# zhb94430/RayTracer-Utah

Hardware: AMD Instinct MI355X
Metric: Mrays/sec at 1920x1080 (the reference's primary + secondary + shadow rays of the frames rendered / wall time; batched throughput: config.frames_in_flight frames with their own cameras per launch sequence — one frame alone: config.single_frame) (higher is better)
Workload: dtype f32

## Files before the change

### raytracer-utah_amd/csrc/render_impl.h

```cpp
#ifndef RTU_RENDER_IMPL_H_INCLUDED
#define RTU_RENDER_IMPL_H_INCLUDED
#include "rtu_intersect.h"

namespace {

#define TEXD ((TEX & 1) != 0)
#define SMPD ((TEX & 2) != 0)
#define BATD ((TEX & 4) != 0)
#define GID ((TEX & 8) != 0)
#define CNTD ((TEX & 16) != 0)
#ifndef RTU_OCC_PRIMARY
#define RTU_OCC_PRIMARY __attribute__((amdgpu_waves_per_eu(4, 4)))
#endif
#ifndef RTU_OCC_PRIMARY_S
#define RTU_OCC_PRIMARY_S __attribute__((amdgpu_waves_per_eu(5, 5)))
#endif
#ifndef RTU_OCC_TRACE
#define RTU_OCC_TRACE __attribute__((amdgpu_waves_per_eu(5, 5)))
#endif
#ifndef RTU_OCC_WALK
#define RTU_OCC_WALK __attribute__((amdgpu_waves_per_eu(3, 3)))
#endif
#ifndef RTU_OCC_CONSUME
#define RTU_OCC_CONSUME
// ... 336 lines not shown
                const int hmid = hit ? as_const(s.nodes)[h.node].material_id : -1;
                a.gi_h[ho] = make_float4(h.p.x, h.p.y, h.p.z, h.z);
                a.gi_h[ho + a.gi_total] = make_float4(h.N.x, h.N.y, h.N.z, __uint_as_float((hit ? 1u : 0u) | (h.front ? 2u : 0u) | ((uint32_t)(hmid + 1) << 2)));
                a.gi_h[ho + 2u * (size_t)a.gi_total] = make_float4(ray.dir.x, ray.dir.y, ray.dir.z, __uint_as_float(smp.key));
                if (TEXD) a.gi_h[ho + 3u * (size_t)a.gi_total] = make_float4(h.uvw.x, h.uvw.y, h.uvw.z, 0.0f);
                RTU_BYTES(TEXD ? 64u : 48u);
            }
        }
        return;
    }
    if (valid) {
        float ox = 0.5f, oy = 0.5f;
        if (smp.on) {
            smp.key = sample_key((uint32_t)x + (uint32_t)a.frame.width * (uint32_t)y, a.sample_index + sidx);
            ox = a.pix_off_x[sidx];
            oy = a.pix_off_y[sidx];
            const float sampleX = (float)rand31(smp.key, RTU_DRAW_LENS) / RTU_RAND_MAX_F;
            const float sampleTheta = (float)rand31(smp.key, RTU_DRAW_LENS + 1u) / RTU_THETA_DIV;
            float sn, cs;
            portable_sincos(sampleTheta, sn, cs);
            const float rad = sqrtf((sampleX * a.frame.dof) * a.frame.dof);
            const float camOffsetX = rad * cs, camOffsetY = rad * sn;
            ray.p = (ray.p + ld3(a.frame.lens_up) * camOffsetY) + ld3(a.frame.lens_right) * camOffsetX;
        }
        f3 cp = (cam_origin + cam_u * ((float)x + ox)) + cam_v * ((float)y + oy);
        ray.dir = norm3(cp - ray.p);
        RTU_CNT(prim);
        bool hit = false;
        const unsigned units0 = CNTD ? cnt.t_inner4 * 2u + cnt.t_tri : 0u;
        if (!(a.dbg & 4u)) hit = trace<STACK, STATS, !STATS, DEFER, COOP, TEXD, CNTD>(s, ray, false, h, stk, cnt, deferred, stride, lds_nodes, skip, rects);
        if (CNTD) walk_units = cnt.t_inner4 * 2u + cnt.t_tri - units0;
        if (!deferred && leader) {
            if (!hit) {
                f3 bg = background_sample<TEXD>(s, x, y);
                if (!(a.dbg & 16u)) a.out[pix] = make_float4(bg.x, bg.y, bg.z, h.z);
                RTU_BYTES(16u);
            } else {
                RTU_CNT(prim_hit);
                mid = as_const(s.nodes)[h.node].material_id;
                if (mid < 0) { a.out[pix] = make_float4(1.0f, 1.0f, 1.0f, h.z); RTU_BYTES(16u); }
                else want = true;
            }
            if (GID) {
                a.gi_h[pix] = make_float4(h.p.x, h.p.y, h.p.z, h.z);
                a.gi_h[pix + a.gi_total] = make_float4(h.N.x, h.N.y, h.N.z, __uint_as_float((want ? 1u : 0u) | (h.front ? 2u : 0u) | ((uint32_t)(mid + 1) << 2)));
                a.gi_h[pix + 2u * (size_t)a.gi_total] = make_float4(ray.dir.x, ray.dir.y, ray.dir.z, __uint_as_float(smp.key));
                if (TEXD) a.gi_h[pix + 3u * (size_t)a.gi_total] = make_float4(h.uvw.x, h.uvw.y, h.uvw.z, 0.0f);
                RTU_BYTES(TEXD ? 64u : 48u);
                want = false;
            }
        }
    }
    if (GID) return;
    uint32_t info = 0;
    if (want) info = make_info<TEX>(a, mid, a.frame.max_bounce, h.front, ray.dir, h.p, h.N, h.uvw, smp);
    if (!STATS && INLINE_SHADE && !(a.dbg & 2048u) && __any(want && !(info & (RTU_FI_MAIN | RTU_FI_C)))) {
        const bool tryI = want && !(info & (RTU_FI_MAIN | RTU_FI_C));
        uint32_t lit = ~0u;
        bool ok = false;
        if (tryI) ok = shadows_inline<TEX>(a, info, h.p, lit, cnt);
        if (tryI && ok) {
            f3 direct = mk3(0, 0, 0);
            if (info & RTU_FI_SH) {
                const f3 cam_pos = BATD ? ld3(a.cam[sidx].pos) : ld3(a.frame.cam_pos);
                direct = direct_light<false, TEX>(a, info, h.p, h.N, h.uvw, cam_pos, direct, [&](uint32_t j) { return ((lit >> j) & 1u) ? 1.0f : 0.0f; });
            }
            a.out[pix] = make_float4(direct.x, direct.y, direct.z, h.z);
            RTU_BYTES(16u);
            want = false;
        }
    }
    if (!(a.dbg & 8u)) append_root<TEX>(a, want, shard, info, h.p, h.N, pix, ray.dir, h.z, h.uvw, cnt, !DEFER && !STATS);
    if (CNTD && !DEFER && !COOP && (a.dbg & 131072u) && valid) a.out[pix].x = (float)walk_units;
}

template <int STACK, bool STATS, int TEX>
__device__ __forceinline__ void primary_stage1(const KernelArgs& a, uint32_t n_tiles) {
    const Stamp stamp(a, RTU_TL_PRIMARY);
    __shared__ uint32_t s_stack_all[STATS ? 4 * STACK * 64 : 4];
    uint32_t* stk = s_stack_all + (STATS ? (threadIdx.x >> 6) * (STACK * 64) + (threadIdx.x & 63u) : 0);
    const uint32_t lane = threadIdx.x & 63u;
    Counters cnt = {};
    const uint32_t wave = (uint32_t)__builtin_amdgcn_readfirstlane((int)(threadIdx.x >> 6));
    for (uint32_t btile = blockIdx.x * 4u + wave; btile < n_tiles; btile += gridDim.x * 4u) {
        uint32_t sidx = (SMPD || BATD) ? btile / a.tiles_per_image : 0u;
        uint32_t tile = btile - sidx * a.tiles_per_image;
        bool lane_on = true;
        if constexpr (SMPD) {
            if (a.act_list != nullptr) {
                sidx = btile / a.act_n;
                const RTU_CONST uint32_t* ent = as_const(reinterpret_cast<const uint32_t*>(a.act_list)) + 4u * (size_t)(btile - sidx * a.act_n);
                tile = ent[0];
                lane_on = (((unsigned long long)ent[3] << 32 | ent[2]) >> lane) & 1ull;
            }
        }
        const uint32_t band_local = tile / a.tiles_x;
        const uint32_t tx = tile - band_local * a.tiles_x;
        const int x = (int)(tx * 8 + (lane & 7));
        const int ly = (int)(band_local * RTU_BAND_ROWS + (lane >> 3));
        const int y = (int)((band_local * a.frame.shard_count + a.frame.shard_rank) * RTU_BAND_ROWS + (lane >> 3));
        const bool valid = x < a.frame.width && y < a.frame.height && lane_on;
        const uint32_t pix = ((SMPD || BATD) ? sidx * a.batch_pixels : 0u) + (uint32_t)ly * (uint32_t)a.frame.width + (uint32_t)x;
        if (!STATS && !SMPD && !GID && a.occ != nullptr) {
            const uint32_t w = as_const(a.occ)[(size_t)sidx * a.occ_words + (tile >> 5)];
            if (!((w >> (tile & 31u)) & 1u)) {
                if (valid) {
                    const f3 bg = background_sample<TEXD>(a.scene, x, y);
                    a.out[pix] = make_float4(bg.x, bg.y, bg.z, RTU_BIGFLOAT);
                    RTU_BYTES(16u);
                    if (CNTD) cnt.t_rays++;
                }
                if (CNTD && lane == 0) cnt.t_bytes += 4u;
                continue;
            }
        }
        const uint32_t shard = btile % RTU_SHARDS;
        bool deferred;
        primary_pixel<STACK, STATS, !STATS, false, TEX, RTU_INLINE_PRIMARY>(a, valid, x, y, sidx, pix, shard, stk, cnt, deferred);
        if (!STATS && !(a.dbg & 8u)) defer_push(a, 0, shard, deferred, pix);
        if (deferred) RTU_BYTES(4u);
    }
    flush_counters<STATS>(a, cnt);
    flush_touched<TEX>(a, cnt, RTU_TL_PRIMARY);
}
template <int STACK, bool STATS, int TEX>
__global__ void __launch_bounds__(256) RTU_OCC_PRIMARY k_primary(KernelArgs a, uint32_t n_tiles) { primary_stage1<STACK, STATS, TEX>(a, n_tiles); }
template <int STACK, int TEX>
__global__ void __launch_bounds__(256) RTU_OCC_PRIMARY_S k_primary_sampled(KernelArgs a, uint32_t n_tiles) { primary_stage1<STACK, false, TEX>(a, n_tiles); }
template <int STACK, int TEX>
__global__ void __launch_bounds__(256) k_primary_counting(KernelArgs a, uint32_t n_tiles) { primary_stage1<STACK, true, TEX>(a, n_tiles); }

__device__ __forceinline__ void stage_nodes(const KernelArgs& a, float4* lds_nodes) {
    const RTU_CONST DevMesh* meshes = as_const(a.scene.meshes);
    for (uint32_t m = 0; m < a.n_meshes; m++) {
        const float4* src = meshes[m].bvh8;
        const uint32_t n = meshes[m].lds_nodes * 16u, off = meshes[m].lds_off;
        for (uint32_t i = threadIdx.x; i < n; i += blockDim.x) lds_nodes[off + i] = src[i];
    }
    __syncthreads();
}

template <int STACK, int TEX>
__global__ void __launch_bounds__(64) RTU_OCC_WALK k_primary2(KernelArgs a, int alone) {
    const Stamp stamp(a, RTU_TL_PRIMARY2);
    __shared__ uint32_t s_stack[STACK * 64];
    const uint32_t lane = threadIdx.x;
    const NarrowGeom g = narrow_geom(a, 0);
    if (g.R == 8u && !alone) return;
    const uint32_t kmax = (g.nmax + 63u) / 64u;
    const uint32_t chunks = kmax * RTU_SHARDS;
    Counters cnt = {};
    const uint32_t counts = g.counts;
    for (uint32_t c = blockIdx.x; c < chunks; c += gridDim.x) {
        const uint32_t shard = c % RTU_SHARDS, k = c / RTU_SHARDS;
        const uint32_t ns = count_of(counts, shard);
        const uint32_t e = k * 64u + lane;
        const bool valid = e < ns;
        uint32_t pix = 0;
        if (valid) pix = a.defer_list0[(size_t)shard * a.defer_cap0_s + e];
        if (valid) RTU_BYTES(4u);
        int x, y;
        uint32_t sidx;
        pixel_of<TEX>(a, pix, x, y, sidx);
        bool deferred;
        primary_pixel<STACK, false, false, false, TEX, RTU_INLINE_PRIMARY2>(a, valid, x, y, sidx, pix, shard, s_stack + lane, cnt, deferred);
    }
    flush_touched<TEX>(a, cnt, RTU_TL_PRIMARY2);
}

template <int STACK, int TEX>
__global__ void __launch_bounds__(RTU_COOP_THREADS) k_primary2c(KernelArgs a, int alone) {
    const Stamp stamp(a, RTU_TL_PRIMARY2C);
    __shared__ float4 s_nodes[RTU_LDS_NODE_F4];
    __shared__ uint32_t s_stack[RTU_COOP_GROUPS * RTU_STACK8];
    const NarrowGeom g = narrow_geom(a, 0);
    if (g.R != 8u && !alone) return;
    const uint32_t grp = threadIdx.x >> 3;
    const bool leader = (threadIdx.x & 7u) == 0;
    const uint32_t groups = g.sum < 12288u ? 32u : (uint32_t)RTU_COOP_GROUPS;
    const uint32_t kmax = (g.nmax + groups - 1u) / groups;
    const uint32_t chunks = kmax * RTU_SHARDS;
    if (blockIdx.x >= chunks) return;
    stage_nodes(a, s_nodes);
    if (grp >= groups) return;
    Counters cnt = {};
    for (uint32_t c = blockIdx.x; c < chunks; c += gridDim.x) {
        const uint32_t shard = c % RTU_SHARDS, k = c / RTU_SHARDS;
        const uint32_t ns = count_of(g.counts, shard);
        const uint32_t e = k * groups + grp;
        const bool valid = e < ns;
        uint32_t pix = 0;
        if (valid) pix = a.defer_list0[(size_t)shard * a.defer_cap0_s + e];
        if (valid && leader) RTU_BYTES(4u);
        int x, y;
        uint32_t sidx;
        pixel_of<TEX>(a, pix, x, y, sidx);
        bool deferred;
        primary_pixel<RTU_STACK8, false, false, true, TEX>(a, valid, x, y, sidx, pix, shard, s_stack + grp, cnt, deferred, leader, RTU_COOP_GROUPS, s_nodes);
    }
    flush_touched<TEX>(a, cnt, RTU_TL_PRIMARY2C);
}

template <int STACK, bool STATS, bool DEFER, bool COOP, int TEX>
// ... 933 lines not shown
__global__ void __launch_bounds__(256) k_prelude(KernelArgs a, uint32_t entries) {
    const uint32_t nm = a.cover ? entries * a.scene.n_cover : 0u, np = a.cover ? entries * a.scene.n_pcover : 0u;
    if (blockIdx.y < nm) mesh_cover_body(a, entries, blockIdx.y);
    else if (blockIdx.y < nm + np) plane_cover_body(a, entries, blockIdx.y - nm);
    else if (blockIdx.x == 0u) node_rects_body(a, entries);
}

__global__ void __launch_bounds__(64) k_tile_occ(KernelArgs a, uint32_t entries) {
    const uint32_t e = blockIdx.y;
    if (e >= entries) return;
    const DevScene& s = a.scene;
    const uint32_t tiles = a.tiles_per_image;
    const uint32_t tile = blockIdx.x * 64u + threadIdx.x;
    bool occ = false;
    if (tile < tiles) {
        const uint32_t band_local = tile / a.tiles_x, tx = tile - band_local * a.tiles_x;
        const int x0 = (int)(tx * 8u), y0 = (int)((band_local * (uint32_t)a.frame.shard_count + (uint32_t)a.frame.shard_rank) * RTU_BAND_ROWS);
        const int x1 = x0 + 8 < a.frame.width ? x0 + 8 : a.frame.width, y1 = y0 + 8 < a.frame.height ? y0 + 8 : a.frame.height;
        const uint32_t gtile = (uint32_t)(y0 >> 3) * a.tiles_xf + tx;
        for (uint32_t k = 0; k < s.n_nodes && k < 64u; k++) {
            if (!((s.obj_mask >> k) & 1ull)) continue;
            const int4 r = a.node_rects[(size_t)e * s.n_nodes + k];
            if (!(x0 < r.z && x1 > r.x && y0 < r.w && y1 > r.y)) continue;
            bool masked_out = false;
            if (a.cover)
                for (uint32_t c = 0; c < s.n_cover + s.n_pcover; c++)
                    if ((uint32_t)(c < s.n_cover ? s.cover_node[c] : s.pcover_node[c - s.n_cover]) == k) {
                        const uint32_t* m = a.cover + ((size_t)e * (s.n_cover + s.n_pcover) + c) * (1u + a.cover_words);
                        if (m[0] == 0u && !((m[1u + (gtile >> 5)] >> (gtile & 31u)) & 1u)) masked_out = true;
                    }
            if (!masked_out) occ = true;
        }
    }
    const unsigned long long bits = __ballot(occ);
    if (threadIdx.x == 0) {
        uint32_t* o = const_cast<uint32_t*>(a.occ) + (size_t)e * a.occ_words + 2u * blockIdx.x;
        o[0] = (uint32_t)bits;
        o[1] = (uint32_t)(bits >> 32);
        if (bits) atomicAdd(&a.fcnt->occ_tiles[((blockIdx.x + 7u * blockIdx.y) % RTU_SHARDS) * RTU_CSTRIDE], (uint32_t)__popcll(bits));
    }
}

#define RTU_LAUNCH_ON(strm_, kslot_, kernel, grid, blk, ...)                                  \
    do {                                                                                     \
        const bool probed_ = probe && probe->slot == (kslot_);                               \
        if (a.host_launches) a.host_launches[(kslot_)]++;                                    \
        if (probed_) (void)hipEventRecord((hipEvent_t)probe->ev0, (strm_));                  \
        hipLaunchKernelGGL(kernel, grid, blk, 0, (strm_), __VA_ARGS__);                      \
        if (probed_) { (void)hipEventRecord((hipEvent_t)probe->ev1, (strm_)); if (probe->recorded) *probe->recorded = 1; } \
    } while (0)
#define RTU_LAUNCH(kslot_, kernel, grid, blk, ...) RTU_LAUNCH_ON(stream, kslot_, kernel, grid, blk, __VA_ARGS__)

template <int STACK, int TEX>
int launch_all(const KernelArgs& a, uint32_t n_tiles, bool stats, hipStream_t stream, int mode = RTU_LAUNCH_ALL, const LaunchProbe* probe = nullptr) {
    const int levels = a.frame.max_bounce + 1;
    const dim3 block(64);
    const dim3 gridT(32768), gridN(32768), gridS(8192), gridF0(16384), gridF(4096), gridC(1024), gridCoop(512);
    const uint32_t thr = (uint32_t)(a.frame.coop_threshold > 0 ? a.frame.coop_threshold : 70000);
    auto grid_lane = [&](int ph, dim3 full) {
        const uint32_t n1 = ph < 8 ? a.list_n[ph] : 0u;
        if (n1 == 0u || n1 - 1u > thr) return full;
        uint32_t g = ((n1 - 1u + 63u) / 64u) * 2u;
        g = g < 2048u ? 2048u : g;
        return g < full.x ? dim3(g) : full;
    };
    auto grid_coop = [&](int ph) {
        const uint32_t n1 = ph < 8 ? a.list_n[ph] : 0u;
        return (n1 != 0u && n1 - 1u > 2u * (uint64_t)thr) ? dim3(16) : gridCoop;
    };
    auto grid_coop2 = [&](int ph) {
        const uint32_t n1 = ph < 8 ? a.list_n[ph] : 0u;
        return (n1 != 0u && n1 - 1u > 2u * (uint64_t)thr) ? dim3(32) : dim3(2u * gridCoop.x);
    };
    auto no_coop = [&](int ph) {
        const uint32_t n1 = ph < 8 ? a.list_n[ph] : 0u;
        return (a.side || !(a.dbg & 16384u)) && n1 != 0u && n1 - 1u > (uint64_t)thr;
    };
    auto no_lane = [&](int ph) {
        const uint32_t n1 = ph < 8 ? a.list_n[ph] : 0u;
        return !(a.dbg & 16384u) && n1 != 0u && (uint64_t)(n1 - 1u) <= (uint64_t)thr - thr / 8u;
    };
    if (n_tiles == 0) return (int)hipSuccess;
    const uint32_t blocksP = (n_tiles + 3) / 4;
    const uint32_t pcap = a.pgrid ? a.pgrid : 32768u;
    const dim3 gridP(blocksP), gridPF(blocksP < pcap ? blocksP : pcap);
    if (CNTD) stats = false;
    if (mode == RTU_LAUNCH_SHADE) {
        RTU_LAUNCH(RTU_TL_GI_ROOTS, (k_gi_roots<TEX>), gridN, block, a, (stats || (a.dbg & 2048u)) ? 0 : 1);
    } else if (stats) {
        if constexpr (!CNTD) hipLaunchKernelGGL((k_primary_counting<STACK, TEX>), gridP, dim3(256), 0, stream, a, n_tiles);
    } else {
        if (!SMPD && a.node_rects) {
            const uint32_t entries = BATD ? a.batch : 1u;
            const uint32_t rows = (a.cover ? entries * (a.scene.n_cover + a.scene.n_pcover) : 0u) + 1u;
            uint32_t gx = 1u;
            if (a.cover && a.scene.n_cover) gx = (a.cover_faces + 255u) / 256u > gx ? (a.cover_faces + 255u) / 256u : gx;
            if (a.cover && a.scene.n_pcover) gx = (a.cover_words * 32u + 255u) / 256u > gx ? (a.cover_words * 32u + 255u) / 256u : gx;
            hipLaunchKernelGGL(k_prelude, dim3(gx, rows), dim3(256), a.cover ? a.cover_words * sizeof(uint32_t) : 0, stream, a, entries);
        }
        if (!SMPD && !GID && a.occ) hipLaunchKernelGGL(k_tile_occ, dim3(a.occ_words / 2u, (BATD ? a.batch : 1u)), dim3(64), 0, stream, a, (BATD ? a.batch : 1u));
        if constexpr (SMPD || GID) RTU_LAUNCH(RTU_TL_PRIMARY, (k_primary_sampled<STACK, TEX>), gridPF, dim3(256), a, n_tiles);
        else RTU_LAUNCH(RTU_TL_PRIMARY, (k_primary<STACK, false, TEX>), gridPF, dim3(256), a, n_tiles);
        if (a.n_meshes && a.side && mode == RTU_LAUNCH_ALL) {
            KernelArgs a2 = a;
            for (int L = 0; L < RTU_MAX_LEVELS; L++) a2.lv[L] = a.lv_side[L];
            a2.fcnt = a.fcnt0;
            const hipStream_t aux = (hipStream_t)a.aux_stream;
            (void)hipEventRecord((hipEvent_t)a.aux_ev0, stream);
            (void)hipStreamWaitEvent(aux, (hipEvent_t)a.aux_ev0, 0);
            {
                const KernelArgs& a = a2;
                RTU_LAUNCH_ON(aux, RTU_TL_PRIMARY2, (k_primary2<STACK, TEX>), grid_lane(0, gridN), block, a, 1);
                RTU_LAUNCH_ON(aux, RTU_TL_SIDE_TAIL, (k_tail<TEX>), dim3(1024), block, a, 0, (int)RTU_TL_SIDE_TAIL);
            }
            (void)hipEventRecord((hipEvent_t)a.aux_ev1, aux);
        } else if (a.n_meshes) {
            const bool nc = no_coop(0), nl = no_lane(0);
            if (!nc) RTU_LAUNCH(RTU_TL_PRIMARY2C, (k_primary2c<STACK, TEX>), grid_coop(0), dim3(RTU_COOP_THREADS), a, nl ? 1 : 0);
            if (!nl) RTU_LAUNCH(RTU_TL_PRIMARY2, (k_primary2<STACK, TEX>), grid_lane(0, gridN), block, a, nc ? 1 : 0);
        }
    }
    if (mode == RTU_LAUNCH_CHAIN) return (int)hipGetLastError();
    const int regular = (!stats && a.tail_from >= 1 && a.tail_from < levels) ? a.tail_from : levels;
    for (int L = 0; L < regular; L++) {
        const int ph = 1 + L;
        if (stats) {
            if constexpr (!CNTD) {
                hipLaunchKernelGGL((k_trace_counting<STACK, TEX>), gridT, block, 0, stream, a, L, (int)(SEL_SHADOW | SEL_MAIN | SEL_C), ph);
                if (L + 1 < levels) hipLaunchKernelGGL((k_trace_counting<STACK, TEX>), gridT, block, 0, stream, a, L, (int)(SEL_A | SEL_A_NEEDS_B), ph);
                hipLaunchKernelGGL((k_consume<true, TEX>), gridF, block, 0, stream, a, L);
            }
        } else {
            const int sel = (int)(SEL_SHADOW | SEL_MAIN | SEL_A | SEL_C);
            RTU_LAUNCH(RTU_TL_LEVEL0 + 4 * L, (k_trace<STACK, false, TEX>), L == 0 ? gridT : gridS, block, a, L, sel, ph);
            if (a.n_meshes) {
                const bool nc = no_coop(ph), nl = no_lane(ph);
                if (!nc) RTU_LAUNCH(RTU_TL_LEVEL0 + 4 * L + 1, (k_trace2c<STACK, TEX>), grid_coop2(ph), dim3(RTU_COOP2_THREADS), a, L, sel, ph, nl ? 1 : 0);
                if (!nl) RTU_LAUNCH(RTU_TL_LEVEL0 + 4 * L + 2, (k_trace2<STACK, TEX>), grid_lane(ph, L == 0 ? gridN : gridS), block, a, L, sel, ph, nc ? 1 : 0);
            }
            RTU_LAUNCH(RTU_TL_LEVEL0 + 4 * L + 3, (k_consume<false, TEX>), L == 0 ? gridF0 : gridF, block, a, L);
        }
    }
    if (regular < levels) RTU_LAUNCH(RTU_TL_LEVEL0 + 4 * regular, (k_tail<TEX>), dim3(8192), block, a, regular, RTU_TL_LEVEL0 + 4 * regular);
    for (int L = regular - 2 + (regular < levels ? 1 : 0); L >= 0; L--) RTU_LAUNCH(RTU_TL_COMBINE0 + L, (k_combine<TEX>), gridC, block, a, L);
    if (!stats && a.n_meshes && a.side && mode == RTU_LAUNCH_ALL) (void)hipStreamWaitEvent(stream, (hipEvent_t)a.aux_ev1, 0);
    return (int)hipGetLastError();
}

}

#endif
```

### raytracer-utah_amd/csrc/rtu_capi.hip

```cpp
#include "rtu_devbuf.h"
#include "rtu_device.h"
#include "rtu_lightlist.h"
#include "rtu_meshrec.h"

#include <algorithm>
#include <array>
#include <cmath>
#include <cstdarg>
#include <cstdio>
#include <cstdlib>
#include <cstring>
#include <map>
#include <memory>
#include <string>
#include <vector>

struct RtuProgressive;

struct RtuContext {
    int         device = 0;
    hipStream_t stream = nullptr;
    hipStream_t aux_stream = nullptr;
    hipEvent_t  aux_ev0 = nullptr, aux_ev1 = nullptr;
    hipEvent_t  ev0 = nullptr, ev1 = nullptr;
// ... 966 lines not shown
    if ((rc = alloc_level(ctx, &ctx->defer_list0, cap_s0_alloc * RTU_SHARDS)) != RTU_OK) return rc;
    ctx->defer_cap0_s = (uint32_t)cap_s0_alloc;
    for (int L = 0; L < RTU_MAX_LEVELS; L++)
        if ((rc = alloc_level_set(ctx, ctx->lv_side[L], 256, false)) != RTU_OK) return rc;
    ctx->level_nsl = ctx->nsl;
    return RTU_OK;
}

float halton(int index, int base) {
    float r = 0;
    float f = 1.0f / (float)base;
    for (int i = index; i > 0; i /= base) {
        r += f * (float)(i % base);
        f /= (float)base;
    }
    return r;
}

int launch(RtuContext* ctx, const RtuFrameDesc* frame, float4* d_out, hipStream_t stream, bool zero_counters, int sample_index = 0, int batch = 1,
           const RtuFrameDesc* frames_batch = nullptr, int gi_mode = RTU_LAUNCH_ALL, int gi_depth = 0, bool adaptive = false,
           const uint4* act_list = nullptr, uint32_t act_n = 0) {
    uint32_t tiles_x = (uint32_t)((frame->width + 7) / 8);
    uint32_t bands = (uint32_t)shard_bands(frame->height, frame->shard_rank, frame->shard_count);
    uint32_t n_tiles = tiles_x * bands * (uint32_t)batch;
    uint32_t pixels = (uint32_t)rtu_shard_rows(frame) * (uint32_t)frame->width;
    const bool gi = gi_mode != RTU_LAUNCH_ALL;
    int rc = ensure_levels(ctx, gi ? 2u * (n_tiles + RTU_SHARDS) : n_tiles, gi);
    if (rc != RTU_OK) return rc;
    if (gi) {
        const size_t chains = (size_t)pixels * (size_t)batch;
        RTU_HIP(ctx, ctx->gi_h.grow(chains * (RTU_GI_BOUNCES + 1) * 4));
        RTU_HIP(ctx, ctx->gi_res.grow(chains * 2));
        if (act_list && gi_mode == RTU_LAUNCH_CHAIN && gi_depth == 0)
            RTU_HIP(ctx, hipMemsetAsync(ctx->gi_h.get() + chains, 0, chains * sizeof(float4), stream));
    }
    const int stats = frame->collect_stats;
    if (stats && zero_counters) {
        RTU_HIP(ctx, hipMemsetAsync(ctx->counters.get(), 0, kCounterBytes, stream));
        memset(ctx->slot_launches, 0, sizeof ctx->slot_launches);
    }
    RTU_HIP(ctx, hipMemsetAsync(ctx->fcnt.get(), 0, offsetof(FrameCounters, overflow), stream));
    KernelArgs a;
    memset(&a, 0, sizeof a);
    a.scene = ctx->dscene;
    a.frame = *frame;
    if (!ctx->any_recursive_material) a.frame.max_bounce = 0;
    a.out = d_out;
    memcpy(a.lv, ctx->lv, sizeof a.lv);
    a.fcnt = ctx->fcnt.get();
    a.tl = ctx->stamp_next ? ctx->tl.get() : nullptr;
    a.defer_list = ctx->defer_list;
    a.defer_cap_s = ctx->defer_cap_s;
    a.defer_list0 = ctx->defer_list0;
    a.defer_cap0_s = ctx->defer_cap0_s;
    a.fcnt0 = ctx->fcnt.get();
    a.dbg = ctx->dbg;
    a.scene.dbg = ctx->dbg;
    a.counters = stats ? ctx->counters.get() : nullptr;
    a.host_launches = stats == 2 ? ctx->slot_launches : nullptr;
    a.node_rects = (stats != 1 && frame->samples == 0 && ctx->dscene.node_bounds) ? ctx->node_rects : nullptr;
    if (a.node_rects && (ctx->dscene.n_cover + ctx->dscene.n_pcover) && !gi && ((size_t)((frame->width + 7) / 8) * (size_t)((frame->height + 7) / 8) + 31u) / 32u <= 12288u) {
        a.tiles_xf = (uint32_t)((frame->width + 7) / 8);
        a.cover_words = (a.tiles_xf * (uint32_t)((frame->height + 7) / 8) + 31u) / 32u;
        a.cover_faces = ctx->cover_faces;
        const size_t need = (size_t)batch * (ctx->dscene.n_cover + ctx->dscene.n_pcover) * (1u + a.cover_words);
        if (need > ctx->cover.size()) {
            RTU_HIP(ctx, hipStreamSynchronize(stream));
            RTU_HIP(ctx, ctx->cover.grow(need));
        }
        RTU_HIP(ctx, hipMemsetAsync(ctx->cover.get(), 0, need * sizeof(uint32_t), stream));
        a.cover = ctx->cover.get();
    }
    if (a.node_rects && !gi && ctx->dscene.n_nodes <= 64u && stats != 1 && !(ctx->dbg & 256u)) {
        a.occ_words = ((tiles_x * bands + 63u) / 64u) * 2u;
        const size_t need = (size_t)batch * a.occ_words;
        if (need > ctx->occ.size()) {
            RTU_HIP(ctx, hipStreamSynchronize(stream));
            RTU_HIP(ctx, ctx->occ.grow(need));
        }
        a.occ = a.occ_words ? ctx->occ.get() : nullptr;
    }
    a.tiles_x = tiles_x;
    a.tiles_per_image = tiles_x * bands;
    a.nsl = ctx->nsl;
    a.n_meshes = ctx->n_meshes;
    const uint32_t act_tiles = act_n ? act_n * (uint32_t)batch : n_tiles;
    const uint64_t tail_key = adaptive ? ((uint64_t)(32 - __builtin_clz(act_tiles | 1u)) << 8) | (uint64_t)(16 | 2 | (gi ? 8 : 0))
                                       : ((uint64_t)n_tiles << 8) | (uint64_t)((frame->samples ? 2 : 0) | (frames_batch ? 4 : 0) | (gi ? 8 : 0));
    int hint = RTU_MAX_LEVELS;
    bool forced = false;
    if (ctx->tail_hint != 0) { hint = ctx->tail_hint; ctx->tail_hint = 0; forced = true; }
    else if (ctx->tail_hints.count(tail_key)) hint = ctx->tail_hints[tail_key];
    a.tail_from = stats == 1 ? RTU_MAX_LEVELS : hint;
    ctx->last_tail_key = tail_key;
    if (stats == 0 && !gi && !(ctx->dbg & 512u) && ctx->list_hints.count(tail_key)) memcpy(a.list_n, ctx->list_hints[tail_key].data(), sizeof a.list_n);
    if (forced) a.dbg |= 128u;
    if (frame->samples >= 1) {
        const float pixelIncrement = (float)(1.0 / frame->samples);
        a.sampling = 1;
        a.sample_index = (uint32_t)sample_index;
        a.batch = (uint32_t)batch;
        a.batch_pixels = pixels;
        a.tiles_per_image = tiles_x * bands;
        for (int b = 0; b < batch; b++) {
            const int index = sample_index + b;
            const float currentOffset = (float)index * pixelIncrement;
            a.pix_off_x[b] = currentOffset + halton(index, 4);
            a.pix_off_y[b] = currentOffset + halton(index, 5);
        }
    }
    if (frames_batch) {
        a.frame_batch = 1;
        a.batch = (uint32_t)batch;
        a.batch_pixels = pixels;
        a.tiles_per_image = tiles_x * bands;
        if (!ctx->d_cams.get()) {
            RTU_HIP(ctx, ctx->d_cams.grow(RTU_MAX_FRAME_BATCH));
            RTU_HIP(ctx, ctx->h_cams.grow((size_t)RTU_MAX_FRAME_BATCH * RtuContext::kCamSlots));
            for (hipEvent_t& e : ctx->cam_ev) RTU_HIP(ctx, hipEventCreateWithFlags(&e, hipEventDisableTiming));
        }
        const int slot = ctx->cam_slot;
        ctx->cam_slot = (slot + 1) % RtuContext::kCamSlots;
        RTU_HIP(ctx, hipEventSynchronize(ctx->cam_ev[slot]));
        BatchCam* hc = ctx->h_cams.get() + (size_t)slot * RTU_MAX_FRAME_BATCH;
        for (int b = 0; b < batch; b++) {
            memcpy(hc[b].pos, frames_batch[b].cam_pos, sizeof hc[b].pos);
            memcpy(hc[b].origin, frames_batch[b].origin, sizeof hc[b].origin);
            memcpy(hc[b].u, frames_batch[b].u, sizeof hc[b].u);
            memcpy(hc[b].v, frames_batch[b].v, sizeof hc[b].v);
        }
        RTU_HIP(ctx, hipMemcpyAsync(ctx->d_cams.get(), hc, sizeof(BatchCam) * (size_t)batch, hipMemcpyHostToDevice, stream));
        RTU_HIP(ctx, hipEventRecord(ctx->cam_ev[slot], stream));
        a.cam = ctx->d_cams.get();
    }
    if (gi) {
        a.gi_h = ctx->gi_h.get();
        a.gi_res = ctx->gi_res.get();
        a.gi_depth = (uint32_t)gi_depth;
        a.gi_total = pixels * (uint32_t)batch;
    }
    const uint32_t launch_tiles = act_list ? act_n * (uint32_t)batch : n_tiles;
    a.act_list = act_list;
    a.act_n = act_n;
    ctx->last_side = false;
    const uint32_t thr0 = (uint32_t)(frame->coop_threshold > 0 ? frame->coop_threshold : 70000);
    if (stats != 1 && !gi && frame->samples == 0 && ctx->n_meshes > 0 && ctx->mesh_hits_childless && !ctx->stamp_next && !(ctx->dbg & (8192u | 2048u | 64u)) &&
        ctx->dscene.node_bounds && ctx->dscene.lmask &&
        !ctx->side_off.count(tail_key) && ctx->list_hints.count(tail_key) && ctx->list_hints[tail_key][0] - 1u > thr0 &&
        ctx->side_frames.count(tail_key) && ctx->side_frames[tail_key] <= 256u) {
        if (!ctx->aux_stream) {
            int prio_least = 0, prio_greatest = 0;
            RTU_HIP(ctx, hipDeviceGetStreamPriorityRange(&prio_least, &prio_greatest));
            RTU_HIP(ctx, hipStreamCreateWithPriority(&ctx->aux_stream, hipStreamNonBlocking, prio_least));
            RTU_HIP(ctx, hipEventCreateWithFlags(&ctx->aux_ev0, hipEventDisableTiming));
            RTU_HIP(ctx, hipEventCreateWithFlags(&ctx->aux_ev1, hipEventDisableTiming));
        }
        a.side = 1;
        a.fcnt0 = ctx->fcnt_side.get();
        memcpy(a.lv_side, ctx->lv_side, sizeof a.lv_side);
        a.aux_stream = ctx->aux_stream;
        a.aux_ev0 = ctx->aux_ev0;
        a.aux_ev1 = ctx->aux_ev1;
        RTU_HIP(ctx, hipMemsetAsync(ctx->fcnt_side.get(), 0, offsetof(FrameCounters, overflow), stream));
        ctx->last_side = true;
    }
    a.pgrid = 32768u;
// ... 1893 lines not shown
```

### raytracer-utah_amd/csrc/rtu_device.h

```cpp
#ifndef RTU_DEVICE_H_INCLUDED
#define RTU_DEVICE_H_INCLUDED

#include "rtu_render.h"
#include "rtu_vec.h"

__device__ __forceinline__ int cvtt_i32(float v) { return (v > -2147483904.0f && v < 2147483648.0f) ? (int)v : (int)0x80000000; }

#define RTU_CONST __attribute__((address_space(4)))
template <class T> __device__ __forceinline__ const RTU_CONST T* as_const(const T* p) {
#pragma clang diagnostic push
#pragma clang diagnostic ignored "-Wold-style-cast"
    return (const RTU_CONST T*)(p);
#pragma clang diagnostic pop
}

#define RTU_GLOBAL __attribute__((address_space(1)))
typedef float rtu_v4f __attribute__((ext_vector_type(4)));
struct GBase {
    const RTU_GLOBAL char* p;
};
template <class T> __device__ __forceinline__ GBase global_base(const T* ptr) {
    const unsigned long long b = (unsigned long long)ptr;
    const unsigned lo = (unsigned)__builtin_amdgcn_readfirstlane((int)(unsigned)b), hi = (unsigned)__builtin_amdgcn_readfirstlane((int)(unsigned)(b >> 32));
    GBase g;
// ... 69 lines not shown

struct DevTexture {
    int32_t type, width, height, pad;
    const uint8_t* rgb;
    float color1[3], color2[3];
};

struct DevScene {
    const DevNode*     nodes;
    const RtuMaterial* materials;
    const RtuLight*    lights;
    const DevMesh*     meshes;
    const DevTexture*  textures;
    const RtuTexMap*   mat_maps;
    RtuTexMap bg_map, env_map;
    RtuEnvColor bg, env;
    int32_t  img_w, img_h;
    uint32_t textured, pad_tex;
    uint32_t n_nodes, n_lights;
    uint32_t walk_stack_limit;
    float    wscale;
    unsigned long long obj_mask;
    uint32_t nol_ok, n_cover;
    int32_t  cover_node[8];
    const DevLightMask* lmask;
    const float4* cover_box[8];
    uint32_t cover_nf[8];
    uint32_t n_pcover, pad_pc;
    int32_t  pcover_node[RTU_MAX_PCOVER];
    float    pcover_quad[RTU_MAX_PCOVER][4][3];
    uint32_t dbg;
    uint32_t node_bounds;
    float    background[3];
    float    environment[3];
};

#define RTU_MAX_LEVELS        (RTU_MAX_BOUNCE + 1)
#define RTU_MAX_FRAME_BATCH 128
#define RTU_MAX_SHADOW_LIGHTS 13

#define RTU_FI_MTL_MASK   0x3FFFFu
#define RTU_FI_BOUNCE_SH  18
#define RTU_FI_FRONT      (1u << 21)
#define RTU_FI_SH         (1u << 22)
#define RTU_FI_MAIN       (1u << 23)
#define RTU_FI_TIR        (1u << 24)
#define RTU_FI_C          (1u << 25)
#define RTU_FI_NOL_SH     27
#define RTU_FI_NOL_LIGHTS 5u
#define RTU_FI_AMB        (1u << 26)

#define RTU_CH_NONE   (-1)
#define RTU_CH_MISS   (-2)
#define RTU_CH_WHITE  (-3)

struct LevelBuffers {
    float4* fa;
    float4* fb;
    float4* fc;
    float4* fres;
    int4*   fchild;
    float*  fsh;
    float4* fslot;
    float4* fuv;
    float4* fsuv;
    uint32_t* lmain;
    uint32_t* lrefl;
    uint32_t* fpend;
    float4* famb;
    uint32_t cap_s;
    uint32_t pad;
};

#define RTU_COOP_THREADS 1024
#define RTU_COOP_GROUPS  (RTU_COOP_THREADS / 8)
#define RTU_COOP2_THREADS 512
#define RTU_COOP2_GROUPS (RTU_COOP2_THREADS / 8)
#define RTU_STACK8       64
#define RTU_REF8_EMPTY   0x0FFFFFFFu
#define RTU_LDS_NODE_F4  4096

#define RTU_MAX_COVER 8
#define RTU_SHARDS 64
#define RTU_TAIL_LEARN   256u
#define RTU_TAIL_DECLINE 4096u
#define RTU_TL_KERNELS 40
#define RTU_TOUCH_FIELDS 12
#define RTU_TOUCH_STRIDE 16
#define RTU_TL_ENDS 8192u
#define RTU_TL_STRIDE (64u + RTU_TL_ENDS)

#define RTU_CSTRIDE 32u
struct FrameCounters {
    uint32_t n_frames[RTU_MAX_LEVELS][RTU_SHARDS * RTU_CSTRIDE];
    uint32_t n_defer[RTU_MAX_LEVELS + 1][RTU_SHARDS * RTU_CSTRIDE];
    uint32_t n_pending[RTU_MAX_LEVELS][RTU_SHARDS * RTU_CSTRIDE];
    uint32_t n_lmain[RTU_MAX_LEVELS][RTU_SHARDS * RTU_CSTRIDE];
    uint32_t n_lrefl[RTU_MAX_LEVELS][RTU_SHARDS * RTU_CSTRIDE];
    uint32_t occ_tiles[RTU_SHARDS * RTU_CSTRIDE];
    uint32_t stage2_frames[RTU_SHARDS * RTU_CSTRIDE];
    uint32_t overflow;
    uint32_t tail_declined;
    uint32_t pad[30];
};

struct BatchCam {
    float pos[3], origin[3], u[3], v[3];
};

struct KernelArgs {
    DevScene     scene;
    RtuFrameDesc frame;
    float4*      out;
    LevelBuffers lv[RTU_MAX_LEVELS];
    LevelBuffers lv_side[RTU_MAX_LEVELS];
    unsigned long long* tl;
    FrameCounters* fcnt;
    uint32_t*    defer_list;
    uint32_t     defer_cap_s;
    FrameCounters* fcnt0;
    uint32_t*    defer_list0;
    uint32_t     defer_cap0_s, side;
    uint32_t     pgrid, pad_pg;
    void*        aux_stream;
    void*        aux_ev0;
    void*        aux_ev1;
    uint32_t     dbg;
    uint32_t*    cover;
    uint32_t     cover_words, tiles_xf;
    uint32_t     cover_faces, pad_cf;
    int4*        node_rects;
    const uint32_t* occ;
    uint32_t     occ_words, pad_occ;
    unsigned long long* counters;
    uint32_t     tiles_x;
    uint32_t     nsl;
    int32_t      shadow_light[RTU_MAX_SHADOW_LIGHTS];
    float        nol_light[RTU_FI_NOL_LIGHTS][4];
    uint32_t     n_meshes;
    int32_t      tail_from;
    uint32_t     list_n[8];
    uint32_t*    host_launches;
    uint32_t     sampling;
    uint32_t     sample_index;
    uint32_t     batch, batch_pixels, tiles_per_image;
    float        pix_off_x[RTU_MAX_BATCH], pix_off_y[RTU_MAX_BATCH];
    float4*      gi_h;
    float4*      gi_res;
    uint32_t     gi_depth, gi_total;
    uint32_t     frame_batch;
    const BatchCam* cam;
    const uint4* act_list;
    uint32_t     act_n, pad_act;
};

#define RTU_LAUNCH_ALL   0
#define RTU_LAUNCH_CHAIN 1
#define RTU_LAUNCH_SHADE 2
#define RTU_GI_BOUNCES   4
struct LaunchProbe {
    int   slot;
    void* ev0;
    void* ev1;
    int*  recorded;
};
int rtu_launch_frame(const KernelArgs& args, uint32_t n_tiles, uint32_t bvh_stack_needed, int stats, hipStream_t stream, int mode = RTU_LAUNCH_ALL,
                     const LaunchProbe* probe = nullptr);
int rtu_launch_gi_final(const KernelArgs& args, hipStream_t stream);

int rtu_launch_accumulate(const float4* samples, uint32_t batch, float4* acc, uint32_t* hits, uint32_t pixels, bool first, hipStream_t stream);
int rtu_launch_resolve(const float4* acc, const uint32_t* hits, float4* out, uint32_t pixels, uint32_t samples, hipStream_t stream);
struct AdaptiveStep {
    const float4* samples;
    float4* acc;
    float4* sq;
    uint32_t* hits;
    uint8_t* counts;
    const uint4* list_in;
    uint4* list_out;
    uint32_t* n_out;
    const uint32_t* skip_if;
    const uint32_t* skip_if_side;
    uint32_t n_in, batch, first, pixels;
    int32_t width, height, shard_rank, shard_count;
    uint32_t tiles_x, min_samples, increment, max_samples;
    float target;
};
int rtu_launch_adaptive_init(uint4* list, uint32_t tiles, uint32_t tiles_x, int width, int height, int shard_rank, int shard_count, hipStream_t stream);
int rtu_launch_adaptive_step(const AdaptiveStep& p, hipStream_t stream);
int rtu_launch_resolve_counts(const float4* acc, const uint32_t* hits, const uint8_t* counts, float4* out, uint8_t* counts_out, uint32_t pixels, hipStream_t stream);
int rtu_launch_progressive_snapshot(const float4* acc, const uint32_t* hits, const uint8_t* counts, uint32_t n, float4* out, uint8_t* counts_out,
                                    uint32_t pixels, hipStream_t stream);

int rtu_launch_pack_image(const float4* rgbz, unsigned long long pixels, float* z_out, unsigned char* rgb_out, hipStream_t stream);

int rtu_launch_minmax_z(const float4* rgbz, uint32_t pixels_per_frame, uint32_t frames, long long* minmax, hipStream_t stream);
int rtu_launch_pack_output(const float4* rgbz, uint32_t pixels_per_frame, uint32_t frames, const long long* minmax, unsigned char* out, hipStream_t stream);

int rtu_launch_selftest_prims(unsigned long long n_rays, unsigned long long seed, unsigned long long* d_mismatches, hipStream_t stream);
int rtu_launch_selftest_fdiv(unsigned long long n_pairs, unsigned long long seed, unsigned long long* d_mismatches, hipStream_t stream);
int rtu_launch_debug_texcoords(const DevScene& s, int op, const DevTexture* tex, const RtuTexMap* map, const float* in, float* out,
                               unsigned long long n, hipStream_t stream);

#endif
```

Baseline: 60570.

## Group primary tiles per wave and fill empty tiles from one occupancy read

The primary kernel now hands each wave a group of 8 consecutive tiles instead of one. It reads the occupancy word once per group and fills all empty tiles with background in a tight loop using precomputed pointers. It then renders only the occupied tiles by iterating the set bits. This is meant to cut per-tile loop overhead and occupancy lookups and to shrink the grid. The cost is coarser load balance, since one wave may get several occupied tiles while another gets none.

```diff
diff --git a/raytracer-utah_amd/csrc/render_impl.h b/raytracer-utah_amd/csrc/render_impl.h
--- a/raytracer-utah_amd/csrc/render_impl.h
+++ b/raytracer-utah_amd/csrc/render_impl.h
@@ -442,18 +442,7 @@
     const uint32_t lane = threadIdx.x & 63u;
     Counters cnt = {};
     const uint32_t wave = (uint32_t)__builtin_amdgcn_readfirstlane((int)(threadIdx.x >> 6));
-    for (uint32_t btile = blockIdx.x * 4u + wave; btile < n_tiles; btile += gridDim.x * 4u) {
-        uint32_t sidx = (SMPD || BATD) ? btile / a.tiles_per_image : 0u;
-        uint32_t tile = btile - sidx * a.tiles_per_image;
-        bool lane_on = true;
-        if constexpr (SMPD) {
-            if (a.act_list != nullptr) {
-                sidx = btile / a.act_n;
-                const RTU_CONST uint32_t* ent = as_const(reinterpret_cast<const uint32_t*>(a.act_list)) + 4u * (size_t)(btile - sidx * a.act_n);
-                tile = ent[0];
-                lane_on = (((unsigned long long)ent[3] << 32 | ent[2]) >> lane) & 1ull;
-            }
-        }
+    auto render_tile = [&](uint32_t btile, uint32_t sidx, uint32_t tile, bool lane_on) {
         const uint32_t band_local = tile / a.tiles_x;
         const uint32_t tx = tile - band_local * a.tiles_x;
         const int x = (int)(tx * 8 + (lane & 7));
@@ -461,24 +450,94 @@
         const int y = (int)((band_local * a.frame.shard_count + a.frame.shard_rank) * RTU_BAND_ROWS + (lane >> 3));
         const bool valid = x < a.frame.width && y < a.frame.height && lane_on;
         const uint32_t pix = ((SMPD || BATD) ? sidx * a.batch_pixels : 0u) + (uint32_t)ly * (uint32_t)a.frame.width + (uint32_t)x;
-        if (!STATS && !SMPD && !GID && a.occ != nullptr) {
-            const uint32_t w = as_const(a.occ)[(size_t)sidx * a.occ_words + (tile >> 5)];
-            if (!((w >> (tile & 31u)) & 1u)) {
-                if (valid) {
-                    const f3 bg = background_sample<TEXD>(a.scene, x, y);
-                    a.out[pix] = make_float4(bg.x, bg.y, bg.z, RTU_BIGFLOAT);
-                    RTU_BYTES(16u);
-                    if (CNTD) cnt.t_rays++;
-                }
-                if (CNTD && lane == 0) cnt.t_bytes += 4u;
-                continue;
-            }
-        }
         const uint32_t shard = btile % RTU_SHARDS;
         bool deferred;
         primary_pixel<STACK, STATS, !STATS, false, TEX, RTU_INLINE_PRIMARY>(a, valid, x, y, sidx, pix, shard, stk, cnt, deferred);
         if (!STATS && !(a.dbg & 8u)) defer_push(a, 0, shard, deferred, pix);
         if (deferred) RTU_BYTES(4u);
+    };
+    if constexpr (!STATS && !SMPD && !GID) {
+        const uint32_t lg = a.group_log2, gsz = 1u << lg;
+        const uint32_t tpi = a.tiles_per_image;
+        const uint32_t gpi = a.groups_per_image;
+        for (uint32_t unit = blockIdx.x * 4u + wave; unit < n_tiles; unit += gridDim.x * 4u) {
+            const uint32_t sidx = BATD ? unit / gpi : 0u;
+            const uint32_t t0 = (unit - sidx * gpi) << lg;
+            const uint32_t nt = tpi - t0 < gsz ? tpi - t0 : gsz;
+            uint32_t bits = 1u;
+            if (a.occ != nullptr) {
+                const uint32_t full = 0xffffffffu >> (32u - nt);
+                const uint32_t w = as_const(a.occ)[(size_t)sidx * a.occ_words + (t0 >> 5)];
+                bits = (w >> (t0 & 31u)) & full;
+                if (bits != full) {
+                    uint32_t band_local = t0 / a.tiles_x;
+                    uint32_t tx = t0 - band_local * a.tiles_x;
+                    const uint32_t ln = __builtin_amdgcn_mbcnt_hi(~0u, __builtin_amdgcn_mbcnt_lo(~0u, 0u));
+                    uint32_t lx = ln & 7, lrow = ln >> 3;
+                    asm volatile("" : "+v"(lx), "+v"(lrow));
+                    int x = (int)(tx * 8 + lx);
+                    int y = (int)((band_local * a.frame.shard_count + a.frame.shard_rank) * RTU_BAND_ROWS + lrow);
+                    typedef float rgbz_t __attribute__((ext_vector_type(4)));
+                    __attribute__((address_space(1))) rgbz_t* p = (__attribute__((address_space(1))) rgbz_t*)a.out + ((BATD ? sidx * a.batch_pixels : 0u) + (band_local * RTU_BAND_ROWS + lrow) * (uint32_t)a.frame.width + (uint32_t)x);
+                    int width = a.frame.width, height = a.frame.height;
+                    uint32_t tiles_x = a.tiles_x;
+                    int carry = (int)RTU_BAND_ROWS * width - 8 * (int)tiles_x;
+                    int sc8 = a.frame.shard_count * (int)RTU_BAND_ROWS;
+                    asm volatile("" : "+s"(width), "+s"(height), "+s"(tiles_x), "+s"(carry), "+s"(sc8), "+v"(p));
+                    float4 bgc = make_float4(0.0f, 0.0f, 0.0f, RTU_BIGFLOAT);
+                    if (!TEXD) {
+                        const f3 bg = background_sample<TEXD>(a.scene, 0, 0);
+                        bgc = make_float4(bg.x, bg.y, bg.z, RTU_BIGFLOAT);
+                        asm volatile("" : "+v"(bgc.x), "+v"(bgc.y), "+v"(bgc.z), "+v"(bgc.w));
+                    }
+                    for (uint32_t i = 0; i < nt; i++) {
+                        if (!((bits >> i) & 1u)) {
+                            if (x < width && y < height) {
+                                if (TEXD) {
+                                    const f3 bg = background_sample<TEXD>(a.scene, x, y);
+                                    bgc = make_float4(bg.x, bg.y, bg.z, RTU_BIGFLOAT);
+                                }
+                                *p = rgbz_t{bgc.x, bgc.y, bgc.z, bgc.w};
+                                RTU_BYTES(16u);
+                                if (CNTD) cnt.t_rays++;
+                            }
+                            if (CNTD && lane == 0) cnt.t_bytes += 4u;
+                        }
+                        x += 8;
+                        p += 8;
+                        if (++tx == tiles_x) {
+                            tx = 0;
+                            x = (int)lx;
+                            y += sc8;
+                            p += carry;
+                        }
+                    }
+                }
+            }
+            while (bits) {
+                uint32_t u = unit;
+                asm volatile("" : "+s"(u));
+                const uint32_t si = BATD ? u / gpi : 0u;
+                const uint32_t tile = ((u - si * gpi) << lg) + (uint32_t)__builtin_ctz(bits);
+                bits &= bits - 1u;
+                render_tile(si * tpi + tile, si, tile, true);
+            }
+        }
+    } else {
+        for (uint32_t btile = blockIdx.x * 4u + wave; btile < n_tiles; btile += gridDim.x * 4u) {
+            uint32_t sidx = (SMPD || BATD) ? btile / a.tiles_per_image : 0u;
+            uint32_t tile = btile - sidx * a.tiles_per_image;
+            bool lane_on = true;
+            if constexpr (SMPD) {
+                if (a.act_list != nullptr) {
+                    sidx = btile / a.act_n;
+                    const RTU_CONST uint32_t* ent = as_const(reinterpret_cast<const uint32_t*>(a.act_list)) + 4u * (size_t)(btile - sidx * a.act_n);
+                    tile = ent[0];
+                    lane_on = (((unsigned long long)ent[3] << 32 | ent[2]) >> lane) & 1ull;
+                }
+            }
+            render_tile(btile, sidx, tile, lane_on);
+        }
     }
     flush_counters<STATS>(a, cnt);
     flush_touched<TEX>(a, cnt, RTU_TL_PRIMARY);
@@ -1578,8 +1637,10 @@
     };
     if (n_tiles == 0) return (int)hipSuccess;
     const uint32_t blocksP = (n_tiles + 3) / 4;
+    const uint32_t n_groups = (n_tiles / a.tiles_per_image) * a.groups_per_image;
+    const uint32_t blocksG = (n_groups + 3) / 4;
     const uint32_t pcap = a.pgrid ? a.pgrid : 32768u;
-    const dim3 gridP(blocksP), gridPF(blocksP < pcap ? blocksP : pcap);
+    const dim3 gridP(blocksP), gridPS(blocksP < pcap ? blocksP : pcap), gridPF(blocksG < pcap ? blocksG : pcap);
     if (CNTD) stats = false;
     if (mode == RTU_LAUNCH_SHADE) {
         RTU_LAUNCH(RTU_TL_GI_ROOTS, (k_gi_roots<TEX>), gridN, block, a, (stats || (a.dbg & 2048u)) ? 0 : 1);
@@ -1595,8 +1656,8 @@
             hipLaunchKernelGGL(k_prelude, dim3(gx, rows), dim3(256), a.cover ? a.cover_words * sizeof(uint32_t) : 0, stream, a, entries);
         }
         if (!SMPD && !GID && a.occ) hipLaunchKernelGGL(k_tile_occ, dim3(a.occ_words / 2u, (BATD ? a.batch : 1u)), dim3(64), 0, stream, a, (BATD ? a.batch : 1u));
-        if constexpr (SMPD || GID) RTU_LAUNCH(RTU_TL_PRIMARY, (k_primary_sampled<STACK, TEX>), gridPF, dim3(256), a, n_tiles);
-        else RTU_LAUNCH(RTU_TL_PRIMARY, (k_primary<STACK, false, TEX>), gridPF, dim3(256), a, n_tiles);
+        if constexpr (SMPD || GID) RTU_LAUNCH(RTU_TL_PRIMARY, (k_primary_sampled<STACK, TEX>), gridPS, dim3(256), a, n_tiles);
+        else RTU_LAUNCH(RTU_TL_PRIMARY, (k_primary<STACK, false, TEX>), gridPF, dim3(256), a, n_groups);
         if (a.n_meshes && a.side && mode == RTU_LAUNCH_ALL) {
             KernelArgs a2 = a;
             for (int L = 0; L < RTU_MAX_LEVELS; L++) a2.lv[L] = a.lv_side[L];
diff --git a/raytracer-utah_amd/csrc/rtu_capi.hip b/raytracer-utah_amd/csrc/rtu_capi.hip
--- a/raytracer-utah_amd/csrc/rtu_capi.hip
+++ b/raytracer-utah_amd/csrc/rtu_capi.hip
@@ -1072,6 +1072,8 @@
     }
     a.tiles_x = tiles_x;
     a.tiles_per_image = tiles_x * bands;
+    a.group_log2 = (a.occ && !(ctx->dbg & 4096u)) ? (uint32_t)__builtin_ctz((unsigned)RTU_TILE_GROUP) : 0u;
+    a.groups_per_image = (a.tiles_per_image + (1u << a.group_log2) - 1u) >> a.group_log2;
     a.nsl = ctx->nsl;
     a.n_meshes = ctx->n_meshes;
     const uint32_t act_tiles = act_n ? act_n * (uint32_t)batch : n_tiles;
diff --git a/raytracer-utah_amd/csrc/rtu_device.h b/raytracer-utah_amd/csrc/rtu_device.h
--- a/raytracer-utah_amd/csrc/rtu_device.h
+++ b/raytracer-utah_amd/csrc/rtu_device.h
@@ -175,6 +175,10 @@
 
 #define RTU_MAX_COVER 8
 #define RTU_SHARDS 64
+#ifndef RTU_TILE_GROUP
+#define RTU_TILE_GROUP 8
+#endif
+static_assert(RTU_TILE_GROUP >= 1 && RTU_TILE_GROUP <= 32 && (RTU_TILE_GROUP & (RTU_TILE_GROUP - 1)) == 0, "a group of tiles lies inside one occupancy word");
 #define RTU_TAIL_LEARN   256u
 #define RTU_TAIL_DECLINE 4096u
 #define RTU_TL_KERNELS 40
@@ -224,7 +228,8 @@
     uint32_t     cover_faces, pad_cf;
     int4*        node_rects;
     const uint32_t* occ;
-    uint32_t     occ_words, pad_occ;
+    uint32_t     occ_words;
+    uint32_t     group_log2, groups_per_image, pad_groups;
     unsigned long long* counters;
     uint32_t     tiles_x;
     uint32_t     nsl;
```

After: 56690. -6.4%, worse.
